# tgialoimtr/cnn_lstm_ctc_ocr

Hardware: AMD Instinct MI355X
Metric: line-crops/sec (train step) at 32x256 bs=256; CER vs ref (higher is better)
Workload: dtype bf16

## Files before the change

cnn_lstm_ctc_ocr_amd/_lib.py:

```python
import ctypes
import os

import torch

_HERE = os.path.dirname(os.path.abspath(__file__))
LIB_PATH = os.environ.get("OCRK_LIB") or os.path.join(_HERE, "libocrk.so")

OCRK_OK = 0
OCRK_ERR_INVALID_ARG = 1
OCRK_ERR_HIP = 2
OCRK_ERR_INFEASIBLE = 3

F32 = 0
BF16 = 1

_p = ctypes.c_void_p
_i32 = ctypes.c_int
_u32 = ctypes.c_uint
_i64 = ctypes.c_int64
_f32 = ctypes.c_float
_sz = ctypes.c_size_t

SIGNATURES = {
    "ocrk_version": [],
# ... 90 lines not shown
    "ocrk_lstm_fwd_persistent_f32": [_p, _p, _p, _i32, _i32, _i32, _p, _p, _p, _p, _p, _p, _p, _sz, _p],
    "ocrk_lstm_bwd_persistent_f32_supported": [_i32, _i32],
    "ocrk_lstm_bwd_persistent_f32_workspace_size": [_i32, _i32],
    "ocrk_lstm_bwd_persistent_f32": [_p, _p, _i32, _i32, _i32, _p, _p, _p, _p, _p, _p, _p, _p, _sz, _p],
    "ocrk_lstm_bwd_persistent_supported": [_i32, _i32],
    "ocrk_lstm_bwd_persistent_workspace_size": [_i32, _i32],
    "ocrk_lstm_bwd_persistent_slices": [_i32, _i32],
    "ocrk_lstm_bwd_persistent": [_p, _p, _i32, _i32, _i32, _p, _p, _p, _p, _p, _p, _p, _p, _sz, _p],
    "ocrk_lstm_fwd": [_p, _p, _p, _p, _p, _i32, _i32, _i32, _p, _p, _p, _p, _i32, _p],
    "ocrk_lstm_bwd": [_p, _p, _p, _p, _i32, _i32, _i32, _p, _p, _p, _p, _i32, _p],
    "ocrk_gemm_workspace_size": [_i32, _i32, _i32, _i32],
    "ocrk_gemm": [_i32, _i32, _i32, _i32, _i32, _f32, _p, _i64, _i64, _p, _i64, _i64, _p, _i64, _i64,
                  _i32, _p, _i32, _i32, _i32, _i32, _i32, _p, _sz, _p],
    "ocrk_adam": [_p, _p, _p, _p, _i64, _f32, _f32, _f32, _f32, _f32, _p],
    "ocrk_adam_ex": [_p, _p, _p, _p, _i64, _f32, _f32, _f32, _f32, _f32, _u32, _p],
    "ocrk_cast": [_p, _i32, _p, _i32, _i64, _p],
    "ocrk_split_bf16": [_p, _i64, _p, _p, _p],
    "ocrk_permute3": [_p, _i32, _i32, _i32, _i32, _p, _i32, _p],
    "ocrk_strided_copy": [_p, _i64, _i64, _i64, _i64, _p, _i32, _i64, _i64, _p],
    "ocrk_colsum_workspace_size": [_i64, _i32],
    "ocrk_colsum": [_p, _i64, _i32, _i32, _p, _i32, _p, _sz, _p],
    "ocrk_slab_sum_workspace_size": [_i32],
    "ocrk_slab_sum": [_p, _i32, _i32, _i32, _p, _i32, _p, _sz, _p],
    "ocrk_relu_mask": [_p, _p, _i64, _f32, _p, _i32, _p],
    "ocrk_mul_scalar": [_p, _i64, _p, _p],
    "ocrk_mean": [_p, _i32, _p, _p],
    "ocrk_seq_len": [_p, _i32, _p, _p],
    "ocrk_timer_create": [_p],
    "ocrk_timer_record": [_p, _p],
    "ocrk_timer_elapsed": [_p, _p, _p],
    "ocrk_timer_destroy": [_p],
}
_RESTYPE = {"ocrk_last_error": ctypes.c_char_p}
_RESTYPE.update({n: ctypes.c_size_t for n in SIGNATURES if n.endswith("_workspace_size")})
_RESTYPE["ocrk_conv_stats_tiles"] = ctypes.c_size_t
_RESTYPE["ocrk_persistent_flags_size"] = ctypes.c_size_t
_RESTYPE["ocrk_bn_bwd_bias_slab_rows"] = ctypes.c_size_t
_RESTYPE["ocrk_bn_bwd_pooled_bias_slab_rows"] = ctypes.c_size_t
_RESTYPE["ocrk_crc32c"] = ctypes.c_uint32


class OcrkError(RuntimeError):

    def __init__(self, status, message):
        super().__init__(message)
        self.status = status
# ... 122 lines not shown
```

cnn_lstm_ctc_ocr_amd/csrc/tensor_ops.hip:

```cpp
#include "common.h"
#include "reduce.h"
#include "mfma_util.h"

template <typename TI, typename TO>
__global__ void __launch_bounds__(256) cast_kernel(const TI* __restrict__ in, TO* __restrict__ out, int64_t n) {
    for (int64_t i = (int64_t)blockIdx.x * 256 + threadIdx.x; i < n; i += (int64_t)gridDim.x * 256)
        out[i] = from_f32<TO>(to_f32(in[i]));
}

template <typename TI, typename TO>
__global__ void __launch_bounds__(256) permute3_kernel(const TI* __restrict__ in, int d0, int d1, int d2,
                                                       TO* __restrict__ out) {
    const int64_t n = (int64_t)d0 * d1 * d2;
    for (int64_t o = (int64_t)blockIdx.x * 256 + threadIdx.x; o < n; o += (int64_t)gridDim.x * 256) {
        int i2 = (int)(o % d2);
        int64_t t = o / d2;
        int i0 = (int)(t % d0);
        int i1 = (int)(t / d0);
        out[o] = from_f32<TO>(to_f32(in[((int64_t)i0 * d1 + i1) * d2 + i2]));
    }
}

namespace ocrk {
namespace {

__global__ void __launch_bounds__(256)
slab_sum_fused(const float* __restrict__ slab, int nslab, int NC, int ld, float* __restrict__ res,
               float* __restrict__ dst_lo, float* __restrict__ dst_hi, int split, int accumulate) {
    constexpr int RG = 64, CQ = 4, U = 16;
    __shared__ double red[RG][4 * CQ + 1];
    const int cq = threadIdx.x % CQ, rg = threadIdx.x / CQ;
    const int c0 = blockIdx.x * 4 * CQ + 4 * cq;
    double s[4] = {0.0, 0.0, 0.0, 0.0};
    if (c0 < NC) {
        const float* col = slab + c0;
        int i = rg;
        for (; i + (U - 1) * RG < nslab; i += U * RG) {
            f32x4 v[U];
#pragma unroll
            for (int u = 0; u < U; ++u) v[u] = *reinterpret_cast<const f32x4*>(col + (int64_t)(i + u * RG) * ld);
#pragma unroll
            for (int u = 0; u < U; ++u)
#pragma unroll
                for (int e = 0; e < 4; ++e) s[e] += v[u][e];
        }
        for (; i < nslab; i += RG) {
            const f32x4 v = *reinterpret_cast<const f32x4*>(col + (int64_t)i * ld);
#pragma unroll
            for (int e = 0; e < 4; ++e) s[e] += v[e];
        }
    }
#pragma unroll
    for (int e = 0; e < 4; ++e) red[rg][4 * cq + e] = s[e];
    __syncthreads();
    if (threadIdx.x < 4 * CQ) {
        const int c = blockIdx.x * 4 * CQ + threadIdx.x;
        if (c >= NC) return;
        double t = 0.0;
        for (int y = 0; y < RG; ++y) t += red[y][threadIdx.x];
        const float v = (float)t;
        if (res) res[c] = v;
        float* d = c < split ? (dst_lo ? dst_lo + c : nullptr) : (dst_hi ? dst_hi + (c - split) : nullptr);
        if (d) *d = accumulate ? *d + v : v;
    }
}

__global__ void __launch_bounds__(256)
slab_sum_stage1(const float* __restrict__ slab, int nslab, int NC, int ld, double* __restrict__ part) {
    __shared__ double red[4][64];
    const int cl = threadIdx.x & 63, q = threadIdx.x >> 6;
    const int c = blockIdx.x * 64 + cl;
    const int rows = (nslab + SLAB_P - 1) / SLAB_P;
    const int r0 = blockIdx.y * rows, r1 = min(nslab, r0 + rows);
    double s = 0.0;
    if (c < NC)
        for (int i = r0 + q; i < r1; i += 4) s += slab[(int64_t)i * ld + c];
    red[q][cl] = s;
    __syncthreads();
    if (q == 0 && c < NC) part[(int64_t)blockIdx.y * NC + c] = red[0][cl] + red[1][cl] + red[2][cl] + red[3][cl];
}

__global__ void __launch_bounds__(64)
slab_sum_stage2(const double* __restrict__ part, int NC, float* __restrict__ res, float* __restrict__ dst_lo,
                float* __restrict__ dst_hi, int split, int accumulate) {
    const int c = blockIdx.x * 64 + threadIdx.x;
    if (c >= NC) return;
    double t = 0.0;
// ... 124 lines not shown
    int64_t rpb = ocrk::cdiv(M, nb);
    nb = std::max<int64_t>(1, ocrk::cdiv(M, rpb));
    hipStream_t s = ocrk::as_stream(stream);
    dim3 grid(colsum_col_blocks(N), (unsigned)nb);
    if (dtype == OCRK_BF16) colsum_partial_kernel<bf16><<<grid, 256, 0, s>>>((const bf16*)in, M, N, rpb, (float*)ws);
    else colsum_partial_kernel<float><<<grid, 256, 0, s>>>((const float*)in, M, N, rpb, (float*)ws);
    int st = ocrk::launch_status("ocrk_colsum");
    if (st) return st;
    double* part = (double*)((char*)ws + ((size_t)nb * N * sizeof(float) + 7) / 8 * 8);
    return ocrk::slab_sum((const float*)ws, (int)nb, N, part, nullptr, out, nullptr, N, accumulate, s);
}

extern "C" size_t ocrk_slab_sum_workspace_size(int nc) { return (size_t)ocrk::SLAB_P * std::max(nc, 1) * sizeof(double); }

extern "C" int ocrk_slab_sum(const float* slab, int nslab, int nc, int ld, float* out, int accumulate, void* ws,
                             size_t ws_bytes, void* stream) {
    OCRK_REQUIRE(nslab >= 0 && nc >= 0 && ld >= nc, "ocrk_slab_sum: bad sizes");
    OCRK_REQUIRE(ws_bytes >= ocrk_slab_sum_workspace_size(nc), "ocrk_slab_sum: workspace too small");
    if (nc == 0) return OCRK_OK;
    return ocrk::slab_sum(slab, nslab, nc, (double*)ws, nullptr, out, nullptr, nc, accumulate, ocrk::as_stream(stream),
                          ld);
}

extern "C" int ocrk_relu_mask(const float* dy, const float* y, int64_t n, float scale, void* out, int out_dtype,
                              void* stream) {
    if (n == 0) return OCRK_OK;
    hipStream_t s = ocrk::as_stream(stream);
    if (out_dtype == OCRK_BF16) relu_mask_kernel<bf16><<<grid1d(n), 256, 0, s>>>(dy, y, n, scale, (bf16*)out);
    else relu_mask_kernel<float><<<grid1d(n), 256, 0, s>>>(dy, y, n, scale, (float*)out);
    return ocrk::launch_status("ocrk_relu_mask");
}

template <typename TO>
__global__ void __launch_bounds__(256) strided_copy_kernel(const float* __restrict__ in, int64_t rows, int64_t cols,
                                                           int64_t in_rs, int64_t in_cs, TO* __restrict__ out,
                                                           int64_t out_rs, int64_t out_cs) {
    const int64_t n = rows * cols;
    for (int64_t i = (int64_t)blockIdx.x * 256 + threadIdx.x; i < n; i += (int64_t)gridDim.x * 256) {
        int64_t r = i / cols, c = i - r * cols;
        out[r * out_rs + c * out_cs] = from_f32<TO>(in[r * in_rs + c * in_cs]);
    }
}

extern "C" int ocrk_strided_copy(const float* in, int64_t rows, int64_t cols, int64_t in_rs, int64_t in_cs,
                                 void* out, int out_dtype, int64_t out_rs, int64_t out_cs, void* stream) {
    int64_t n = rows * cols;
// ... 164 lines not shown
```

cnn_lstm_ctc_ocr_amd/kernels.py:

```python
import ctypes

import torch

from . import _lib, options
from ._lib import ptr, call

F32, BF16 = _lib.F32, _lib.BF16
_DT = {torch.float32: F32, torch.bfloat16: BF16}


def dtype_code(dt):
    try:
        return _DT[dt]
    except KeyError:
        raise TypeError(f"unsupported dtype {dt}; libocrk computes in float32 or bfloat16")


def _stream(t):
    return _lib.stream_ptr(t.device)


def _chk(*ts):
    for t in ts:
        if t is None:
# ... 139 lines not shown
    _chk(x, w_nk, bias, stats)
    B, H, W, Cin = x.shape
    Cout = w_nk.shape[0]
    y_dtype = y_dtype or x.dtype
    y = torch.empty(B, H, W, Cout, dtype=y_dtype, device=x.device)
    call("ocrk_conv3x3_fwd", ptr(x), B, H, W, Cin, ptr(w_nk), ptr(bias), Cout, ptr(y), dtype_code(y_dtype),
         int(relu), ptr(stats), dtype_code(x.dtype), _stream(x))
    return y


def conv3x3_bwd_data(dy, w_bwd, relu_mask=None, dbias=None, accumulate=True, defer=None, relu_bits=None):
    _chk(dy, w_bwd, relu_mask, dbias, relu_bits)
    B, H, W, Cout = dy.shape
    Cin = w_bwd.shape[0]
    dx = torch.empty(B, H, W, Cin, dtype=dy.dtype, device=dy.device)
    if relu_bits is not None:
        if relu_mask is not None:
            raise ValueError("relu_bits replaces relu_mask")
        if dbias is not None and defer is not None:
            tiles = conv_stats_tiles(B * H * W)
            slab = torch.empty(tiles, 2 * Cin, dtype=torch.float32, device=dy.device)
            call("ocrk_conv3x3_bwd_data_bits_slab", ptr(dy), B, H, W, Cout, ptr(w_bwd), Cin, ptr(dx), ptr(relu_bits),
                 ptr(slab), dtype_code(dy.dtype), _stream(dy))
            defer.append((lambda: slab_sum(slab, tiles, Cin, 2 * Cin, dbias, accumulate), (slab,)))
            return dx
        nb, ws = 0, None
        if dbias is not None:
            nb = _lib.lib().ocrk_conv3x3_bwd_data_workspace_size(B, H, W, Cin)
            ws = _ws(nb, dy.device)
        call("ocrk_conv3x3_bwd_data_bits", ptr(dy), B, H, W, Cout, ptr(w_bwd), Cin, ptr(dx), ptr(relu_bits),
             ptr(dbias), int(accumulate), ptr(ws), nb, dtype_code(dy.dtype), _stream(dy))
        return dx
    if dbias is not None and defer is not None:
        tiles = conv_stats_tiles(B * H * W)
        slab = torch.empty(tiles, 2 * Cin, dtype=torch.float32, device=dy.device)
        call("ocrk_conv3x3_bwd_data_slab", ptr(dy), B, H, W, Cout, ptr(w_bwd), Cin, ptr(dx), ptr(relu_mask),
             ptr(slab), dtype_code(dy.dtype), _stream(dy))
        defer.append((lambda: slab_sum(slab, tiles, Cin, 2 * Cin, dbias, accumulate), (slab,)))
        return dx
    nb, ws = 0, None
    if dbias is not None:
        nb = _lib.lib().ocrk_conv3x3_bwd_data_workspace_size(B, H, W, Cin)
        ws = _ws(nb, dy.device)
    call("ocrk_conv3x3_bwd_data", ptr(dy), B, H, W, Cout, ptr(w_bwd), Cin, ptr(dx), ptr(relu_mask), ptr(dbias),
         int(accumulate), ptr(ws), nb, dtype_code(dy.dtype), _stream(dy))
    return dx


def conv3x3_bwd_weight(x, dy, dw, accumulate=True):
    _chk(x, dy, dw)
    B, H, W, Cin = x.shape
    Cout = dy.shape[-1]
    nb = _lib.lib().ocrk_conv3x3_wgrad_workspace_size(B, H, W, Cin, Cout)
    ws = _ws(nb, x.device)
    call("ocrk_conv3x3_bwd_weight", ptr(x), ptr(dy), B, H, W, Cin, Cout, ptr(dw), int(accumulate), ptr(ws), nb,
         dtype_code(x.dtype), _stream(x))


def bn_finalize(stats, M, C, eps, momentum, moving_mean=None, moving_var=None, tile_rows=128):
    _chk(stats, moving_mean, moving_var)
    tiles = stats.shape[0]
# ... 66 lines not shown
                     dbias=None, defer=None, sync=None, pooled=None):
    _chk(z, dp, mean, invstd, gamma, beta, dgamma, dbeta, dbias, pooled)
    B, H, W, C = z.shape
    kh, kw, sh, sw = pool
    nb = _lib.lib().ocrk_bn_bwd_workspace_size(B, H, W, C)
    ws = _ws(nb, z.device)
    dz = torch.empty_like(z)
    if sync is not None:
        return _bn_bwd_sync(z, dp, mean, invstd, gamma, beta, pool, dp_time_major, dgamma, dbeta, accumulate, dbias,
                            defer, sync, dz, ws, nb)
    if pooled is not None:
        if pooled.shape != dp.shape or pooled.dtype != dp.dtype:
            raise ValueError("pooled must have dp's shape and dtype")
        rows = _lib.lib().ocrk_bn_bwd_pooled_bias_slab_rows(B, H, W, C, kh, kw, sh, sw)
        if rows == 0:
            pooled = None
    if pooled is not None:
        slab = None
        if dbias is not None and defer is not None:
            slab = torch.empty(rows, 2 * C, dtype=torch.float32, device=z.device)
        call("ocrk_bn_relu_pool_bwd_pooled", ptr(z), ptr(pooled), ptr(dp), B, H, W, C, ptr(mean), ptr(invstd),
             ptr(gamma), ptr(beta), kh, kw, sh, sw, int(dp_time_major), ptr(dz), ptr(dgamma), ptr(dbeta),
             ptr(dbias), int(accumulate), ptr(slab), ptr(ws), nb, dtype_code(z.dtype), _stream(z))
        if slab is not None:
            def _late():
                slab_sum(slab, rows, C, 2 * C, dbias, accumulate)
                slab_sum(slab.view(-1)[C:], rows, C, 2 * C, dgamma, accumulate)
            defer.append((_late, (slab,)))
        return dz
    if dbias is not None and defer is not None:
        rows = _lib.lib().ocrk_bn_bwd_bias_slab_rows(B, H, W, C, kh, kw, sh, sw)
        slab = torch.empty(rows, C, dtype=torch.float32, device=z.device)
        call("ocrk_bn_relu_pool_bwd_slab", ptr(z), ptr(dp), B, H, W, C, ptr(mean), ptr(invstd), ptr(gamma),
             ptr(beta), kh, kw, sh, sw, int(dp_time_major), ptr(dz), ptr(dgamma), ptr(dbeta), int(accumulate),
             ptr(slab), ptr(ws), nb, dtype_code(z.dtype), _stream(z))
        defer.append((lambda: slab_sum(slab, rows, C, C, dbias, accumulate), (slab,)))
        return dz
    call("ocrk_bn_relu_pool_bwd", ptr(z), ptr(dp), B, H, W, C, ptr(mean), ptr(invstd), ptr(gamma), ptr(beta),
         kh, kw, sh, sw, int(dp_time_major), ptr(dz), ptr(dgamma), ptr(dbeta), ptr(dbias), int(accumulate),
         ptr(ws), nb,
         dtype_code(z.dtype), _stream(z))
    return dz


def _bn_bwd_sync(z, dp, mean, invstd, gamma, beta, pool, dp_time_major, dgamma, dbeta, accumulate, dbias, defer,
                 sync, dz, ws, nb):
    import torch.distributed as dist
    group, count = sync
    B, H, W, C = z.shape
    kh, kw, sh, sw = pool
    dsum = torch.empty(2 * C, dtype=torch.float32, device=z.device)
    args = (ptr(z), ptr(dp), B, H, W, C, ptr(mean), ptr(invstd), ptr(gamma), ptr(beta), kh, kw, sh, sw,
            int(dp_time_major))
    call("ocrk_bn_relu_pool_bwd_reduce", *args, ptr(dgamma), ptr(dbeta), int(accumulate), ptr(dsum), ptr(ws), nb,
         dtype_code(z.dtype), _stream(z))
    dist.all_reduce(dsum, op=dist.ReduceOp.SUM, group=group)
    slab = None
    if dbias is not None and defer is not None:
        rows = _lib.lib().ocrk_bn_bwd_bias_slab_rows(B, H, W, C, kh, kw, sh, sw)
        slab = torch.empty(rows, C, dtype=torch.float32, device=z.device)
    call("ocrk_bn_relu_pool_bwd_apply", *args, ptr(dsum), ptr(count), ptr(dz),
         ptr(dbias if slab is None else None), int(accumulate), ptr(slab), ptr(ws), nb, dtype_code(z.dtype), _stream(z))
    if slab is not None:
        defer.append((lambda: slab_sum(slab, rows, C, C, dbias, accumulate), (slab,)))
    return dz


def gemm(a, b, trans_a=False, trans_b=False, bias=None, relu=False, out=None, out_dtype=torch.float32,
         accumulate=False, alpha=1.0, M=None, N=None, K=None, lda=None, ldb=None, ldc=None,
         batch=1, stride_a=0, stride_b=0, stride_c=0, splits=1):
    for t in (a, b, bias, out):
        if t is not None and not t.is_cuda:
            raise ValueError("libocrk ops take device tensors (got a CPU tensor)")
    if M is None:
        _chk(a, b)
        M, K = (a.shape[1], a.shape[0]) if trans_a else (a.shape[0], a.shape[1])
        N = b.shape[0] if trans_b else b.shape[1]
        lda, ldb = a.shape[1], b.shape[1]
    if out is None:
        out = torch.empty(M, N, dtype=out_dtype, device=a.device)
        ldc = N
    ldc = ldc if ldc is not None else N
    if a.dtype != b.dtype:
        raise TypeError("gemm operands must share a dtype")
    kc = -(-(-(-K // splits)) // 32) * 32 if splits > 1 else K
    splits = -(-K // kc) if splits > 1 else 1
    nb = _lib.lib().ocrk_gemm_workspace_size(M, N, batch, splits) if splits > 1 else 0
# ... 292 lines not shown
    _chk(table, stream_of)
    call("ocrk_copy_batch", ptr(table), int(njobs), int(total_tiles), _stream(stream_of))


def strided_copy(src, rows, cols, in_rs, in_cs, out, out_rs, out_cs, out_offset=0, in_offset=0):
    _chk(src, out)
    sp = ctypes_offset(src, in_offset)
    op = ctypes_offset(out, out_offset)
    call("ocrk_strided_copy", sp, rows, cols, in_rs, in_cs, op, dtype_code(out.dtype), out_rs, out_cs, _stream(src))


def ctypes_offset(t, elems):
    return ctypes.c_void_p(t.data_ptr() + elems * t.element_size())


def slab_sum(slab, nslab, nc, ld, out, accumulate=True):
    _chk(slab, out)
    nb = _lib.lib().ocrk_slab_sum_workspace_size(nc)
    ws = _ws(nb, slab.device)
    call("ocrk_slab_sum", ptr(slab), int(nslab), int(nc), int(ld), ptr(out), int(accumulate), ptr(ws), nb,
         _stream(slab))


def _bias_parts(part, rows, nc, dbias, defer):
    if defer is None:
        slab_sum(part, rows, nc, nc, dbias)
    else:
        defer.append((lambda: slab_sum(part, rows, nc, nc, dbias), (part,)))


def colsum(x, M, N, out, accumulate=True):
    _chk(x, out)
    nb = _lib.lib().ocrk_colsum_workspace_size(M, N)
    ws = _ws(nb, x.device)
    call("ocrk_colsum", ptr(x), M, N, dtype_code(x.dtype), ptr(out), int(accumulate), ptr(ws), nb, _stream(x))


def relu_mask(dy, y, out_dtype, scale=1.0):
    _chk(dy, y)
    out = torch.empty(dy.shape, dtype=out_dtype, device=dy.device)
    call("ocrk_relu_mask", ptr(dy), ptr(y), dy.numel(), float(scale), ptr(out), dtype_code(out_dtype), _stream(dy))
    return out


def mul_scalar_(x, s):
    _chk(x, s)
    call("ocrk_mul_scalar", ptr(x), x.numel(), ptr(s), _stream(x))
    return x


def mean(x):
# ... 174 lines not shown
```

cnn_lstm_ctc_ocr_amd/model.py:

```python
import contextlib

import numpy as np
import torch
import torch.distributed as dist

from . import kernels as K
from . import options
from .config import BN_EPS, BN_MOMENTUM, INFER, LAYER_PARAMS, POOLS, TRAIN, ModelConfig, rnn_size
from .params import ParamStore

layer_params = LAYER_PARAMS

_DEFAULT = []


@contextlib.contextmanager
def use_store(store):
    _DEFAULT.append(store)
    try:
        yield store
    finally:
        _DEFAULT.pop()


# ... 92 lines not shown
                                             store.stats[pe + "/batch_norm/moving_variance"], BN_EPS)
        p = K.bn_relu_pool_fwd(z, mean, invstd, P[pe + "/batch_norm/gamma"], P[pe + "/batch_norm/beta"],
                               POOLS[even], time_major=(k == 4))
        ctx.store, ctx.k = store, k
        ctx.save_for_backward(x, y_odd, z, mean, invstd, p)
        return p

    @staticmethod
    def backward(ctx, dp):
        with _conv_precision(ctx.exact):
            return _ConvBlock._backward(ctx, dp)

    @staticmethod
    def _backward(ctx, dp):
        store, k = ctx.store, ctx.k
        x, y_odd, z, mean, invstd, pooled = ctx.saved_tensors
        dt = store.cfg.dtype
        P, G = store.params, store.grads
        odd, even = f"conv{2 * k - 1}", f"conv{2 * k}"
        pe, po = f"convnet/{even}", f"convnet/{odd}"
        dp = dp.contiguous()
        if dp.dtype != dt:
            dp = K.cast(dp, dt)
        dz = K.bn_relu_pool_bwd(z, dp, mean, invstd, P[pe + "/batch_norm/gamma"], P[pe + "/batch_norm/beta"],
                                POOLS[even], dp_time_major=(k == 4),
                                dgamma=G[pe + "/batch_norm/gamma"], dbeta=G[pe + "/batch_norm/beta"],
                                dbias=G[pe + "/bias"],
                                sync=ctx.bn_sync,
                                pooled=pooled if ctx.bn_sync is None and ctx.pooled_bn else None)
        B, H, W, C = dz.shape
        if k > 1:
            with _conv_side(store, y_odd, dz, *_conv_late_tensors(store)):
                _conv_late_run(store)
                _conv_wgrad(ctx.exact, y_odd, dz, G[pe + "/kernel"])
        _, w_bwd = store.conv_images(even, dt)
        if ctx.conv12_bwd:
            if store.conv_late:
                with _conv_side(store, *_conv_late_tensors(store)):
                    _conv_late_run(store)
            K.conv12_bwd(dz, w_bwd, x, P["convnet/conv1/kernel"], P["convnet/conv1/bias"], G[pe + "/kernel"],
                         G[po + "/kernel"], G[po + "/bias"], relu_bits=ctx.relu_bits)
            store.join()
            return (None, None, None, None) + (None,) * (len(ctx.needs_input_grad) - 4)
        if ctx.c1_fused and K.conv2_bwd_data_conv1_wgrad_ok(dz, x):
            with _conv_side(store, y_odd, dz, *_conv_late_tensors(store)):
                _conv_late_run(store)
                _conv_wgrad(ctx.exact, y_odd, dz, G[pe + "/kernel"])
            bits = ctx.relu_bits
            K.conv2_bwd_data_conv1_wgrad(dz, w_bwd, None if bits is not None else y_odd, x, G[po + "/kernel"],
                                         G[po + "/bias"], relu_bits=bits)
            store.join()
            return (None, None, None, None) + (None,) * (len(ctx.needs_input_grad) - 4)
        if k > 1 and ctx.relu_bits is not None:
            dy_odd = K.conv3x3_bwd_data(dz, w_bwd, dbias=G[po + "/bias"], relu_bits=ctx.relu_bits)
        else:
            dy_odd = K.conv3x3_bwd_data(dz, w_bwd, relu_mask=y_odd, dbias=G[po + "/bias"] if k > 1 else None)
        dx = None
        if k == 1:
            with _conv_side(store, x, dy_odd, *_conv_late_tensors(store)):
                _conv_late_run(store)
                K.conv1_bwd_weight(x, dy_odd, G[po + "/kernel"], G[po + "/bias"])
            _conv_wgrad(ctx.exact, y_odd, dz, G[pe + "/kernel"])
            store.join()
        else:
            if k > 2 and options.get("CONV_SIDE") and options.get("SIDE_STREAM"):
                store.conv_late.append((lambda x=x, d=dy_odd, dw=G[po + "/kernel"], ex=ctx.exact:
                                        _conv_wgrad(ex, x, d, dw), (x, dy_odd)))
            else:
                with _conv_side(store, x, dy_odd):
                    _conv_wgrad(ctx.exact, x, dy_odd, G[po + "/kernel"])
            if ctx.needs_input_grad[0]:
                _, w_bwd_odd = store.conv_images(odd, dt)
                dx = K.conv3x3_bwd_data(dy_odd, w_bwd_odd)
        return (dx, None, None, None) + (None,) * (len(ctx.needs_input_grad) - 4)


def _bn_group(store):
    g = store.bn_group
    if g is None or not (dist.is_available() and dist.is_initialized()):
# ... 93 lines not shown
    @staticmethod
    def forward(ctx, x, seq_len, store, layer, *variables):
        dt = store.cfg.dtype
        T, B, n_in = x.shape
        H = store.cfg.rnn_sizes[layer - 1]
        wxT, _wx, whT, _wh, bias = store.lstm_images(layer, dt)
        gx = K.gemm(x.view(T * B, n_in), wxT, trans_b=True, bias=bias, out_dtype=dt)
        out, hprev, cprev, acts = K.lstm_fwd(gx, whT, seq_len, T, B, H, dt, save=any(ctx.needs_input_grad))
        ctx.store, ctx.layer, ctx.H = store, layer, H
        ctx.save_for_backward(x, seq_len, hprev, cprev, acts)
        return out

    @staticmethod
    def backward(ctx, dout):
        store, layer, H = ctx.store, ctx.layer, ctx.H
        x, seq_len, hprev, cprev, acts = ctx.saved_tensors
        dt = store.cfg.dtype
        T, B, n_in = x.shape
        G4 = 4 * H
        dout = dout.contiguous()
        if dout.dtype != dt:
            dout = K.cast(dout, dt)
        _wxT, wx, _whT, wh, _bias = store.lstm_images(layer, dt)
        dG = K.lstm_bwd(wh, seq_len, dout, cprev, acts, T, B, H, dbias=store.flat_bias_pair_grad(layer))
        R = T * B
        dx = None
        pre = f"rnn/bdrnn{layer}"
        with side_work(store, x, hprev, dG):
            gf, gb = store.grads[f"{pre}/fw/lstm_cell/kernel"], store.grads[f"{pre}/bw/lstm_cell/kernel"]
            sk = gf.numel()
            if dt == torch.float32 and not K.f32_mode_exact():
                (xh, xl), (hh, hl), (gh, gl) = K.split_bf16(x), K.split_bf16(hprev), K.split_bf16(dG)
                passes = [(xh, hh, gh), (xh, hh, gl), (xl, hl, gh)]
            else:
                passes = [(x, hprev, dG)]
            if gb.data_ptr() == gf.data_ptr() + 4 * sk:
                for _xa, ha, ga in passes:
                    K.gemm(ha.view(R, 2 * H), ga.view(R, 2 * G4), trans_a=True, out=gf[n_in:], accumulate=True,
                           M=H, N=G4, K=R, lda=2 * H, ldb=2 * G4, ldc=G4, batch=2, stride_a=H, stride_b=G4,
                           stride_c=sk, splits=_splits(H, G4, R, batch=2, items=_tn_items(layer)))
                for xa, _ha, ga in passes:
                    K.gemm(xa, ga.view(R, 2 * G4), trans_a=True, out=gf, accumulate=True, M=n_in, N=G4, K=R,
                           lda=n_in, ldb=2 * G4, ldc=G4, batch=2, stride_a=0, stride_b=G4, stride_c=sk,
                           splits=_splits(n_in, G4, R, batch=2, items=_tn_items(layer)))
            else:
                for xa, ha, ga in passes:
                    dg = ga.view(R, 2 * G4)
# ... 14 lines not shown
    @staticmethod
    def forward(ctx, x, seq_len, store, layer, *variables):
        dt = store.cfg.dtype
        T, B, n_in = x.shape
        H = store.cfg.rnn_sizes[layer - 1]
        wxT, _wx, whgT, whcT, _whg, _whc, bias = store.gru_images(layer, dt)
        gx = K.gemm(x.view(T * B, n_in), wxT, trans_b=True, bias=bias, out_dtype=dt)
        out, hprev, rh, acts = K.gru_fwd(gx, whgT, whcT, seq_len, T, B, H, dt)
        ctx.store, ctx.layer, ctx.H = store, layer, H
        ctx.save_for_backward(x, seq_len, hprev, rh, acts)
        return out

    @staticmethod
    def backward(ctx, dout):
        store, layer, H = ctx.store, ctx.layer, ctx.H
        x, seq_len, hprev, rh, acts = ctx.saved_tensors
        dt = store.cfg.dtype
        T, B, n_in = x.shape
        G2, G3 = 2 * H, 3 * H
        dout = dout.contiguous()
        if dout.dtype != dt:
            dout = K.cast(dout, dt)
        _wxT, wx, _whgT, _whcT, whg, whc, _bias = store.gru_images(layer, dt)
        dG = K.gru_bwd(whg, whc, seq_len, dout, hprev, acts, T, B, H, dbias=store.gru_bias_cat_grad(layer))
        pre = f"rnn/bdrnn{layer}"
        R = T * B
        side = side_work(store, x, hprev, rh, dG)
        side.__enter__()
        gf, gb = store.grads[f"{pre}/fw/gru_cell/gates/kernel"], store.grads[f"{pre}/bw/gru_cell/gates/kernel"]
        cf, cb = store.grads[f"{pre}/fw/gru_cell/candidate/kernel"], store.grads[f"{pre}/bw/gru_cell/candidate/kernel"]
        sk = (gb.data_ptr() - gf.data_ptr()) // 4
        batched = sk > 0 and cb.data_ptr() - cf.data_ptr() == 4 * sk
        if batched:
            dg = dG.view(R, 2 * G3)
            hp, rhv = hprev.view(R, 2 * H), rh.view(R, 2 * H)
            K.gemm(x, dg, trans_a=True, out=gf, accumulate=True, M=n_in, N=G2, K=R, lda=n_in, ldb=2 * G3,
                   ldc=G2, batch=2, stride_a=0, stride_b=G3, stride_c=sk, splits=_splits(n_in, G2, R, batch=2, items=_tn_items(layer)))
            K.gemm(hp, dg, trans_a=True, out=gf[n_in:], accumulate=True, M=H, N=G2, K=R, lda=2 * H, ldb=2 * G3,
                   ldc=G2, batch=2, stride_a=H, stride_b=G3, stride_c=sk, splits=_splits(H, G2, R, batch=2, items=_tn_items(layer)))
            K.gemm(x, dg[:, G2:], trans_a=True, out=cf, accumulate=True, M=n_in, N=H, K=R, lda=n_in,
                   ldb=2 * G3, ldc=H, batch=2, stride_a=0, stride_b=G3, stride_c=sk,
                   splits=_splits(n_in, H, R, batch=2, items=_tn_items(layer)))
            K.gemm(rhv, dg[:, G2:], trans_a=True, out=cf[n_in:], accumulate=True, M=H, N=H, K=R, lda=2 * H,
                   ldb=2 * G3, ldc=H, batch=2, stride_a=H, stride_b=G3, stride_c=sk, splits=_splits(H, H, R, batch=2, items=_tn_items(layer)))
        for d, dn in enumerate(() if batched else ("fw", "bw")):
            gk = store.grads[f"{pre}/{dn}/gru_cell/gates/kernel"]
            ck = store.grads[f"{pre}/{dn}/gru_cell/candidate/kernel"]
# ... 217 lines not shown
```

cnn_lstm_ctc_ocr_amd/options.py:

```python
import contextlib
import os

_HOST_DEFAULTS = {
    "LSTM_PERSISTENT": 1,
    "F32_TRAIN_EXACT": 0,
    "SIDE_STREAM": 1,
    "CONV_SIDE": 1,
    "CONV12_FUSED": 1,
    "RELU_BITS": 1,
    "POOLED_BN": 1,
    "CONV1_FUSED": 1,
    "CONV12_BWD": 1,
    "TN_ITEMS": 256,
    "TN_ITEMS_L1": 160,
}
KERNEL_OPTIONS = ("CONV_DIRECT", "CONV_ROWS", "CONV_ROWS_WIDE", "CONV_WGRAD_BLOCKS", "LSTM_SPIN_LIMIT",
                  "PERSIST_LATE", "LSTM_BWD_R16", "CTC_LDS",
                  "PP_PERSIST_NK", "NT_F32_EXACT", "NT_F32_MASK",
                  "NT_F32_X6", "BEAM_WAVE", "BN_BWD_BLOCKS", "BN_ROUTE", "BN_ROUTE_SEG", "BN_ROUTE_NCH", "CONV_TN_ITEMS", "CONV_TN4_ITEMS",
                  "CONV_WGRAD_CUS", "F32_MFMA", "GEMM_NT", "GEMM_NT_STAGED", "GEMM_PP", "GEMM_PPTN", "PP_MIN_N", "GEMM_TN",
                  "LSTM_DMA", "LSTM_BWD_DMA", "LSTM_FWD_R16", "NT_TAP_UNIFORM",
                  "GEMM_W4", "GEMM_W4_LAUNCHES")


def _env_int(name, default):
    v = os.environ.get("OCRK_" + name)
    if v is None or v == "":
        return default
    try:
        return int(v)
    except ValueError:
        raise ValueError(f"OCRK_{name}={v!r}: an integer is expected") from None


_HOST = {k: _env_int(k, d) for k, d in _HOST_DEFAULTS.items()}
# ... 41 lines not shown
```

cnn_lstm_ctc_ocr_amd/params.py:

```python

import numpy as np
import torch

from . import kernels as K
from .config import LAYER_PARAMS, ModelConfig

_ALIGN = 64


def param_shapes(cfg):
    out = []
    cin = 1
    for filters, k, _pad, name, bn in LAYER_PARAMS:
        out.append((f"convnet/{name}/kernel", (k, k, cin, filters), True))
        out.append((f"convnet/{name}/bias", (filters,), True))
        if bn:
            out.append((f"convnet/{name}/batch_norm/gamma", (filters,), True))
            out.append((f"convnet/{name}/batch_norm/beta", (filters,), True))
            out.append((f"convnet/{name}/batch_norm/moving_mean", (filters,), False))
            out.append((f"convnet/{name}/batch_norm/moving_variance", (filters,), False))
        cin = filters
    n_in = cin
    for li, H in enumerate(cfg.rnn_sizes, start=1):
        pre = f"rnn/bdrnn{li}"
        if cfg.cell == "lstm":
            for d in ("fw", "bw"):
                out.append((f"{pre}/{d}/lstm_cell/kernel", (n_in + H, 4 * H), True))
# ... 66 lines not shown
        self.offsets = {}
        sizes = {True: 0, False: 0}
        for name, shape, tr in self.spec:
            n = int(np.prod(shape))
            self.offsets[name] = (tr, sizes[tr], shape)
            sizes[tr] += (n + _ALIGN - 1) // _ALIGN * _ALIGN
        self.n_trainable = sum(int(np.prod(s)) for _, s, tr in self.spec if tr)
        self.flat = torch.zeros(sizes[True], dtype=torch.float32, device=self.device)
        self.flat_grad = torch.zeros_like(self.flat)
        self.flat_stats = torch.zeros(max(sizes[False], _ALIGN), dtype=torch.float32, device=self.device)
        self.params, self.grads, self.stats = {}, {}, {}
        for name, shape, tr in self.spec:
            _, off, _ = self.offsets[name]
            n = int(np.prod(shape))
            if tr:
                self.params[name] = self.flat[off:off + n].view(shape)
                self.grads[name] = self.flat_grad[off:off + n].view(shape)
            else:
                self.stats[name] = self.flat_stats[off:off + n].view(shape)
        self.version = 0
        self._images = {}
        self.pending = []
        self.conv_late = []
        self.bn_group = None
        self.f32_conv_exact = False
        self.load_state_dict(values if values is not None else reference_init(self.cfg, seed))

    def state_dict(self):
        out = {k: v.detach().cpu().numpy().copy() for k, v in self.params.items()}
        out.update({k: v.detach().cpu().numpy().copy() for k, v in self.stats.items()})
        return out

    def load_state_dict(self, values):
        for name, _shape, _tr in self.spec:
            if name not in values:
                raise KeyError(f"missing variable {name}")
            dst = self.params.get(name, self.stats.get(name))
            src = torch.as_tensor(np.asarray(values[name], dtype=np.float32))
            if tuple(src.shape) != tuple(dst.shape):
                raise ValueError(f"{name}: shape {tuple(src.shape)} != {tuple(dst.shape)}")
            dst.copy_(src.to(self.device))
        self.bump()

    def save(self, path):
        np.savez(path, **{k.replace("/", "__"): v for k, v in self.state_dict().items()})

    def load(self, path):
        with np.load(path, allow_pickle=False) as z:
            self.load_state_dict({k.replace("__", "/"): z[k] for k in z.files})

    def zero_grad(self):
        self.join()
        self.flat_grad.zero_()

    def join(self):
        while self.conv_late:
            fn, _tensors = self.conv_late.pop(0)
            fn()
        if self.pending:
            cur = torch.cuda.current_stream(self.device)
            for ev in self.pending:
                K.wait_mark(cur, ev)
            self.pending.clear()

    def bump(self):
        self.version += 1
        self._images.clear()
        self._plan_fresh = False

    def images(self, key, builder):
        plan = self._plan_for(key)
        if plan is not None:
            if not self._plan_fresh:
                K.copy_batch(plan["table"], plan["njobs"], plan["tiles"], self.flat)
                self._plan_fresh = True
            return plan["images"][key]
        img = self._images.get(key)
        if img is None:
            img = builder()
            self._images[key] = img
        return img
# ... 193 lines not shown
```

cnn_lstm_ctc_ocr_amd/train.py:

```python
import collections
import math
import time

import torch
import torch.distributed as dist

from . import _lib
from . import kernels as K
from . import options
from . import model as _model
from .config import TRAIN
from .model import check_feasible_host, convnet_layers, ctc_loss_layer, dense_labels, host_labels, rnn_layers




class GradBuckets:

    def __init__(self, store, group=None, comm=None, force=False):
        self.store, self.group, self.comm, self.force = store, group, comm, bool(force)
        rnn = [off for name, (tr, off, _s) in store.offsets.items() if tr and name.startswith("rnn/")]
        self.split = min(rnn) if rnn else store.flat_grad.numel()
        self.work = None
        self._stream = None
        self._comm_world = comm.info()[0] if comm is not None else None

    def world(self):
        if self.comm is not None:
            return self._comm_world
        if not (dist.is_available() and dist.is_initialized()):
            return 1
        return dist.get_world_size(self.group)

    def active(self):
        return self.world() > 1 or (self.force and (self.comm is not None or
                                                    (dist.is_available() and dist.is_initialized())))

    def _sum_(self, t, async_op=False):
        if self.comm is not None:
            self.comm.allreduce_(t)
            return None
        return dist.all_reduce(t, op=dist.ReduceOp.SUM, group=self.group, async_op=async_op)

    def rnn_ready(self, *_):
        if not self.active() or self.work is not None:
            return
        g = self.store.flat_grad
        if g.is_cuda:
            if self._stream is None:
                self._stream = torch.cuda.Stream(g.device)
            K.fork(self._stream, torch.cuda.current_stream(g.device))
            for ev in self.store.pending:
                K.wait_mark(self._stream, ev)
            with torch.cuda.stream(self._stream):
                self.work = self._sum_(g[self.split:], async_op=True)
                if self.work is None:
                    self.work = "stream"
                g.record_stream(self._stream)
        else:
            self.work = self._sum_(g[self.split:], async_op=True)

    def finish(self):
        if not self.active():
            return 1.0
        world = self.world()
        g = self.store.flat_grad
        if self.work is None:
            self._sum_(g)
        else:
            self._sum_(g[:self.split])
# ... 64 lines not shown
        self.buckets = GradBuckets(store, process_group, comm=comm, force=force_exchange)
        self.overlap_allreduce = True

    def learning_rate(self, step=None):
        step = self.global_step if step is None else step
        e = step / self.decay_steps
        if self.staircase:
            e = math.floor(e)
        return self.base_lr * self.decay_rate ** e

    def _bn_group(self):
        if not self.sync_bn or not (dist.is_available() and dist.is_initialized()):
            return None
        return self.group if self.group is not None else dist.group.WORLD

    def world_size(self):
        if self.buckets.comm is not None:
            return self.buckets.world()
        if dist.is_available() and dist.is_initialized():
            return dist.get_world_size(self.group)
        return 1

    def loss_and_grads(self, image, width, label):
        store = self.store
        if store.cfg.dtype != torch.float32:
            return self._loss_and_grads(image, width, label)
        if options.get("F32_TRAIN_EXACT"):
            with K.f32_exact():
                return self._loss_and_grads(image, width, label)
        prev, store.f32_conv_exact = store.f32_conv_exact, True
        try:
            return self._loss_and_grads(image, width, label)
        finally:
            store.f32_conv_exact = prev

    def _loss_and_grads(self, image, width, label):
        store = self.store
        prev_group, store.bn_group = store.bn_group, self._bn_group()
        try:
            return self._forward_backward(image, width, label)
        finally:
            store.bn_group = prev_group

    def _forward_backward(self, image, width, label):
        store = self.store
        if host_labels(label) and not (isinstance(width, torch.Tensor) and width.is_cuda):
# ... 182 lines not shown
```

include/ocrk.h:

```cpp
#ifndef OCRK_H_
#define OCRK_H_

#include <stddef.h>
#include <stdint.h>

#ifdef __cplusplus
extern "C" {
#endif

#define OCRK_ABI_VERSION 7

enum ocrk_status {
    OCRK_OK = 0,
    OCRK_ERR_INVALID_ARG = 1,
    OCRK_ERR_HIP = 2,
    OCRK_ERR_INFEASIBLE = 3
};

enum ocrk_dtype { OCRK_F32 = 0, OCRK_BF16 = 1 };

int ocrk_set_f32_gemm_mode(int mode);
int ocrk_f32_gemm_exact(void);

enum ocrk_device_status {
// ... 211 lines not shown
int ocrk_gemm(int trans_a, int trans_b, int M, int N, int K, float alpha, const void* A, int64_t lda,
              int64_t stride_a, const void* B, int64_t ldb, int64_t stride_b, void* C, int64_t ldc,
              int64_t stride_c, int c_dtype, const float* bias, int relu, int accumulate, int batch,
              int dtype, int splits, void* ws, size_t ws_bytes, void* stream);

int ocrk_adam(float* p, const float* g, float* m, float* v, int64_t n, float lr_t, float beta1,
              float beta2, float eps, float grad_scale, void* stream);
#define OCRK_ADAM_ZERO_GRAD 1u
int ocrk_adam_ex(float* p, float* g, float* m, float* v, int64_t n, float lr_t, float beta1,
                 float beta2, float eps, float grad_scale, unsigned flags, void* stream);

int ocrk_copy_batch(const void* jobs, int njobs, int64_t total_tiles, void* stream);
int ocrk_cast(const void* in, int in_dtype, void* out, int out_dtype, int64_t n, void* stream);
int ocrk_permute3(const void* in, int in_dtype, int d0, int d1, int d2, void* out, int out_dtype,
                  void* stream);
int ocrk_strided_copy(const float* in, int64_t rows, int64_t cols, int64_t in_rs, int64_t in_cs, void* out,
                      int out_dtype, int64_t out_rs, int64_t out_cs, void* stream);
size_t ocrk_colsum_workspace_size(int64_t M, int N);
int ocrk_colsum(const void* in, int64_t M, int N, int dtype, float* out, int accumulate, void* ws,
                size_t ws_bytes, void* stream);
size_t ocrk_slab_sum_workspace_size(int nc);
int ocrk_slab_sum(const float* slab, int nslab, int nc, int ld, float* out, int accumulate, void* ws,
                  size_t ws_bytes, void* stream);
int ocrk_relu_mask(const float* dy, const float* y, int64_t n, float scale, void* out, int out_dtype,
                   void* stream);
int ocrk_mul_scalar(float* x, int64_t n, const float* s, void* stream);
int ocrk_mean(const float* x, int n, float* out, void* stream);
int ocrk_seq_len(const int* widths, int n, int* out, void* stream);

int ocrk_timer_create(void** ev);
int ocrk_timer_record(void* ev, void* stream);
int ocrk_timer_elapsed(void* ev0, void* ev1, float* ms);
int ocrk_timer_destroy(void* ev);

uint32_t ocrk_crc32c(const void* data, size_t n, uint32_t crc);

#ifdef __cplusplus
}
#endif
#endif
```

Before: 56660.

## Batch deferred bias/BN slab reductions into one grouped kernel launch

Adds a batched slab-sum kernel that takes a table of up to 16 reduction jobs and maps blocks to jobs by prefix offsets. The training step now queues bias and gamma slab reductions from the conv, BN-pool and RNN backward passes instead of launching one kernel each, then flushes them once before the gradient all-reduce or join. The goal is to cut many small kernel launches and Python dispatch overhead in backward. In exchange the reductions finish later, the queue holds slabs alive longer, and unaligned items fall back to per-item launches with async malloc and free.

```diff
diff --git a/cnn_lstm_ctc_ocr_amd/_lib.py b/cnn_lstm_ctc_ocr_amd/_lib.py
--- a/cnn_lstm_ctc_ocr_amd/_lib.py
+++ b/cnn_lstm_ctc_ocr_amd/_lib.py
@@ -136,6 +136,7 @@
     "ocrk_colsum": [_p, _i64, _i32, _i32, _p, _i32, _p, _sz, _p],
     "ocrk_slab_sum_workspace_size": [_i32],
     "ocrk_slab_sum": [_p, _i32, _i32, _i32, _p, _i32, _p, _sz, _p],
+    "ocrk_slab_sum_batch": [_p, _i32, _p],
     "ocrk_relu_mask": [_p, _p, _i64, _f32, _p, _i32, _p],
     "ocrk_mul_scalar": [_p, _i64, _p, _p],
     "ocrk_mean": [_p, _i32, _p, _p],
diff --git a/cnn_lstm_ctc_ocr_amd/csrc/tensor_ops.hip b/cnn_lstm_ctc_ocr_amd/csrc/tensor_ops.hip
--- a/cnn_lstm_ctc_ocr_amd/csrc/tensor_ops.hip
+++ b/cnn_lstm_ctc_ocr_amd/csrc/tensor_ops.hip
@@ -24,13 +24,13 @@
 namespace ocrk {
 namespace {
 
-__global__ void __launch_bounds__(256)
-slab_sum_fused(const float* __restrict__ slab, int nslab, int NC, int ld, float* __restrict__ res,
-               float* __restrict__ dst_lo, float* __restrict__ dst_hi, int split, int accumulate) {
+__device__ __forceinline__ void slab_sum_body(const float* __restrict__ slab, int nslab, int NC, int ld,
+                                              float* __restrict__ res, float* __restrict__ dst_lo,
+                                              float* __restrict__ dst_hi, int split, int accumulate, int bx) {
     constexpr int RG = 64, CQ = 4, U = 16;
     __shared__ double red[RG][4 * CQ + 1];
     const int cq = threadIdx.x % CQ, rg = threadIdx.x / CQ;
-    const int c0 = blockIdx.x * 4 * CQ + 4 * cq;
+    const int c0 = bx * 4 * CQ + 4 * cq;
     double s[4] = {0.0, 0.0, 0.0, 0.0};
     if (c0 < NC) {
         const float* col = slab + c0;
@@ -54,7 +54,7 @@
     for (int e = 0; e < 4; ++e) red[rg][4 * cq + e] = s[e];
     __syncthreads();
     if (threadIdx.x < 4 * CQ) {
-        const int c = blockIdx.x * 4 * CQ + threadIdx.x;
+        const int c = bx * 4 * CQ + threadIdx.x;
         if (c >= NC) return;
         double t = 0.0;
         for (int y = 0; y < RG; ++y) t += red[y][threadIdx.x];
@@ -63,6 +63,27 @@
         float* d = c < split ? (dst_lo ? dst_lo + c : nullptr) : (dst_hi ? dst_hi + (c - split) : nullptr);
         if (d) *d = accumulate ? *d + v : v;
     }
+}
+
+__global__ void __launch_bounds__(256)
+slab_sum_fused(const float* __restrict__ slab, int nslab, int NC, int ld, float* __restrict__ res,
+               float* __restrict__ dst_lo, float* __restrict__ dst_hi, int split, int accumulate) {
+    slab_sum_body(slab, nslab, NC, ld, res, dst_lo, dst_hi, split, accumulate, blockIdx.x);
+}
+
+constexpr int SLAB_BATCH = 16;
+struct SlabBatchArgs {
+    OcrkSlabSumItem item[SLAB_BATCH];
+    int first[SLAB_BATCH + 1];
+    int n;
+};
+
+__global__ void __launch_bounds__(256) slab_sum_batch_kernel(const SlabBatchArgs a) {
+    int k = 0;
+    while (k + 1 < a.n && (int)blockIdx.x >= a.first[k + 1]) ++k;
+    const OcrkSlabSumItem& it = a.item[k];
+    slab_sum_body(it.slab, it.nslab, it.nc, it.ld, nullptr, it.dst_lo, it.dst_hi, it.split, it.accumulate,
+                  (int)blockIdx.x - a.first[k]);
 }
 
 __global__ void __launch_bounds__(256)
@@ -233,6 +254,66 @@
                           ld);
 }
 
+namespace {
+bool slab_dst_overlap(const OcrkSlabSumItem& a, const OcrkSlabSumItem& b) {
+    const float* ra[2][2] = {{a.dst_lo, a.dst_lo ? a.dst_lo + a.split : nullptr},
+                             {a.dst_hi, a.dst_hi ? a.dst_hi + (a.nc - a.split) : nullptr}};
+    const float* rb[2][2] = {{b.dst_lo, b.dst_lo ? b.dst_lo + b.split : nullptr},
+                             {b.dst_hi, b.dst_hi ? b.dst_hi + (b.nc - b.split) : nullptr}};
+    for (auto& x : ra)
+        for (auto& y : rb)
+            if (x[0] && y[0] && x[0] < y[1] && y[0] < x[1]) return true;
+    return false;
+}
+
+int slab_batch_launch(ocrk::SlabBatchArgs& a, hipStream_t s) {
+    if (a.n == 0) return OCRK_OK;
+    ocrk::slab_sum_batch_kernel<<<a.first[a.n], 256, 0, s>>>(a);
+    a.n = 0;
+    return ocrk::launch_status("ocrk_slab_sum_batch");
+}
+}
+
+extern "C" int ocrk_slab_sum_batch(const OcrkSlabSumItem* items, int n, void* stream) {
+    OCRK_REQUIRE(n >= 0 && (items || n == 0), "ocrk_slab_sum_batch: n=%d items without a table", n);
+    for (int i = 0; i < n; ++i) {
+        const OcrkSlabSumItem& it = items[i];
+        OCRK_REQUIRE(it.nslab >= 0 && it.nc >= 0 && it.ld >= it.nc && it.split >= 0 && it.split <= it.nc,
+                     "ocrk_slab_sum_batch: item %d has bad sizes (nslab=%d nc=%d ld=%d split=%d)", i, it.nslab,
+                     it.nc, it.ld, it.split);
+        OCRK_REQUIRE(it.slab || it.nslab == 0 || it.nc == 0, "ocrk_slab_sum_batch: item %d has no slab", i);
+    }
+    hipStream_t s = ocrk::as_stream(stream);
+    ocrk::SlabBatchArgs a;
+    a.n = 0;
+    a.first[0] = 0;
+    for (int i = 0; i < n; ++i) {
+        const OcrkSlabSumItem& it = items[i];
+        if (it.nc == 0) continue;
+        const bool fused = it.nc % 4 == 0 && it.ld % 4 == 0 && ((uintptr_t)it.slab & 15) == 0;
+        bool close = !fused || a.n == ocrk::SLAB_BATCH;
+        for (int k = 0; k < a.n && !close; ++k) close = slab_dst_overlap(a.item[k], it);
+        if (close) {
+            int st = slab_batch_launch(a, s);
+            if (st) return st;
+        }
+        if (!fused) {
+            double* part = nullptr;
+            if (hipMallocAsync((void**)&part, ocrk_slab_sum_workspace_size(it.nc), s) != hipSuccess)
+                return ocrk::launch_status("ocrk_slab_sum_batch scratch");
+            int st = ocrk::slab_sum(it.slab, it.nslab, it.nc, part, nullptr, it.dst_lo, it.dst_hi, it.split,
+                                    it.accumulate, s, it.ld);
+            if (hipFreeAsync(part, s) != hipSuccess && !st) st = ocrk::launch_status("ocrk_slab_sum_batch scratch");
+            if (st) return st;
+            continue;
+        }
+        a.item[a.n] = it;
+        a.first[a.n + 1] = a.first[a.n] + (it.nc + 15) / 16;
+        ++a.n;
+    }
+    return slab_batch_launch(a, s);
+}
+
 extern "C" int ocrk_relu_mask(const float* dy, const float* y, int64_t n, float scale, void* out, int out_dtype,
                               void* stream) {
     if (n == 0) return OCRK_OK;
diff --git a/cnn_lstm_ctc_ocr_amd/kernels.py b/cnn_lstm_ctc_ocr_amd/kernels.py
--- a/cnn_lstm_ctc_ocr_amd/kernels.py
+++ b/cnn_lstm_ctc_ocr_amd/kernels.py
@@ -185,7 +185,7 @@
             slab = torch.empty(tiles, 2 * Cin, dtype=torch.float32, device=dy.device)
             call("ocrk_conv3x3_bwd_data_bits_slab", ptr(dy), B, H, W, Cout, ptr(w_bwd), Cin, ptr(dx), ptr(relu_bits),
                  ptr(slab), dtype_code(dy.dtype), _stream(dy))
-            defer.append((lambda: slab_sum(slab, tiles, Cin, 2 * Cin, dbias, accumulate), (slab,)))
+            _defer_sum(defer, slab, tiles, Cin, 2 * Cin, dbias, accumulate)
             return dx
         nb, ws = 0, None
         if dbias is not None:
@@ -199,7 +199,7 @@
         slab = torch.empty(tiles, 2 * Cin, dtype=torch.float32, device=dy.device)
         call("ocrk_conv3x3_bwd_data_slab", ptr(dy), B, H, W, Cout, ptr(w_bwd), Cin, ptr(dx), ptr(relu_mask),
              ptr(slab), dtype_code(dy.dtype), _stream(dy))
-        defer.append((lambda: slab_sum(slab, tiles, Cin, 2 * Cin, dbias, accumulate), (slab,)))
+        _defer_sum(defer, slab, tiles, Cin, 2 * Cin, dbias, accumulate)
         return dx
     nb, ws = 0, None
     if dbias is not None:
@@ -312,7 +312,9 @@
         call("ocrk_bn_relu_pool_bwd_pooled", ptr(z), ptr(pooled), ptr(dp), B, H, W, C, ptr(mean), ptr(invstd),
              ptr(gamma), ptr(beta), kh, kw, sh, sw, int(dp_time_major), ptr(dz), ptr(dgamma), ptr(dbeta),
              ptr(dbias), int(accumulate), ptr(slab), ptr(ws), nb, dtype_code(z.dtype), _stream(z))
-        if slab is not None:
+        if isinstance(defer, SlabSumQueue) and slab is not None:
+            defer.add(slab, rows, 2 * C, 2 * C, dbias, accumulate, dst_hi=dgamma, split=C)
+        elif slab is not None:
             def _late():
                 slab_sum(slab, rows, C, 2 * C, dbias, accumulate)
                 slab_sum(slab.view(-1)[C:], rows, C, 2 * C, dgamma, accumulate)
@@ -324,7 +326,7 @@
         call("ocrk_bn_relu_pool_bwd_slab", ptr(z), ptr(dp), B, H, W, C, ptr(mean), ptr(invstd), ptr(gamma),
              ptr(beta), kh, kw, sh, sw, int(dp_time_major), ptr(dz), ptr(dgamma), ptr(dbeta), int(accumulate),
              ptr(slab), ptr(ws), nb, dtype_code(z.dtype), _stream(z))
-        defer.append((lambda: slab_sum(slab, rows, C, C, dbias, accumulate), (slab,)))
+        _defer_sum(defer, slab, rows, C, C, dbias, accumulate)
         return dz
     call("ocrk_bn_relu_pool_bwd", ptr(z), ptr(dp), B, H, W, C, ptr(mean), ptr(invstd), ptr(gamma), ptr(beta),
          kh, kw, sh, sw, int(dp_time_major), ptr(dz), ptr(dgamma), ptr(dbeta), ptr(dbias), int(accumulate),
@@ -352,7 +354,7 @@
     call("ocrk_bn_relu_pool_bwd_apply", *args, ptr(dsum), ptr(count), ptr(dz),
          ptr(dbias if slab is None else None), int(accumulate), ptr(slab), ptr(ws), nb, dtype_code(z.dtype), _stream(z))
     if slab is not None:
-        defer.append((lambda: slab_sum(slab, rows, C, C, dbias, accumulate), (slab,)))
+        _defer_sum(defer, slab, rows, C, C, dbias, accumulate)
     return dz
 
 
@@ -691,11 +693,56 @@
          _stream(slab))
 
 
+class SlabSumItem(ctypes.Structure):
+    _fields_ = [("slab", ctypes.c_void_p), ("nslab", ctypes.c_int), ("nc", ctypes.c_int), ("ld", ctypes.c_int),
+                ("dst_lo", ctypes.c_void_p), ("dst_hi", ctypes.c_void_p), ("split", ctypes.c_int),
+                ("accumulate", ctypes.c_int)]
+
+
+def slab_sum_batch(items):
+    if not items:
+        return
+    table = (SlabSumItem * len(items))()
+    for e, (slab, nslab, nc, ld, dst_lo, dst_hi, split, accumulate) in zip(table, items):
+        _chk(slab, dst_lo, dst_hi)
+        e.slab, e.nslab, e.nc, e.ld = slab.data_ptr(), int(nslab), int(nc), int(ld)
+        e.dst_lo = None if dst_lo is None else dst_lo.data_ptr()
+        e.dst_hi = None if dst_hi is None else dst_hi.data_ptr()
+        e.split, e.accumulate = int(split), int(accumulate)
+    call("ocrk_slab_sum_batch", table, len(items), _stream(items[0][0]))
+
+
+class SlabSumQueue:
+
+    def __init__(self):
+        self.items = []
+
+    def __len__(self):
+        return len(self.items)
+
+    def add(self, slab, nslab, nc, ld, dst_lo, accumulate=True, dst_hi=None, split=None):
+        self.items.append((slab, nslab, nc, ld, dst_lo, dst_hi, nc if split is None else split, accumulate))
+
+    def flush(self):
+        items, self.items = self.items, []
+        slab_sum_batch(items)
+
+    def clear(self):
+        self.items = []
+
+
+def _defer_sum(defer, slab, nslab, nc, ld, dst, accumulate=True):
+    if isinstance(defer, SlabSumQueue):
+        defer.add(slab, nslab, nc, ld, dst, accumulate)
+    else:
+        defer.append((lambda: slab_sum(slab, nslab, nc, ld, dst, accumulate), (slab,)))
+
+
 def _bias_parts(part, rows, nc, dbias, defer):
     if defer is None:
         slab_sum(part, rows, nc, nc, dbias)
     else:
-        defer.append((lambda: slab_sum(part, rows, nc, nc, dbias), (part,)))
+        _defer_sum(defer, part, rows, nc, nc, dbias)
 
 
 def colsum(x, M, N, out, accumulate=True):
diff --git a/cnn_lstm_ctc_ocr_amd/model.py b/cnn_lstm_ctc_ocr_amd/model.py
--- a/cnn_lstm_ctc_ocr_amd/model.py
+++ b/cnn_lstm_ctc_ocr_amd/model.py
@@ -138,11 +138,12 @@
         dp = dp.contiguous()
         if dp.dtype != dt:
             dp = K.cast(dp, dt)
+        late = store.late_defer()
         dz = K.bn_relu_pool_bwd(z, dp, mean, invstd, P[pe + "/batch_norm/gamma"], P[pe + "/batch_norm/beta"],
                                 POOLS[even], dp_time_major=(k == 4),
                                 dgamma=G[pe + "/batch_norm/gamma"], dbeta=G[pe + "/batch_norm/beta"],
                                 dbias=G[pe + "/bias"],
-                                sync=ctx.bn_sync,
+                                defer=late, sync=ctx.bn_sync,
                                 pooled=pooled if ctx.bn_sync is None and ctx.pooled_bn else None)
         B, H, W, C = dz.shape
         if k > 1:
@@ -168,9 +169,10 @@
             store.join()
             return (None, None, None, None) + (None,) * (len(ctx.needs_input_grad) - 4)
         if k > 1 and ctx.relu_bits is not None:
-            dy_odd = K.conv3x3_bwd_data(dz, w_bwd, dbias=G[po + "/bias"], relu_bits=ctx.relu_bits)
+            dy_odd = K.conv3x3_bwd_data(dz, w_bwd, dbias=G[po + "/bias"], relu_bits=ctx.relu_bits, defer=late)
         else:
-            dy_odd = K.conv3x3_bwd_data(dz, w_bwd, relu_mask=y_odd, dbias=G[po + "/bias"] if k > 1 else None)
+            dy_odd = K.conv3x3_bwd_data(dz, w_bwd, relu_mask=y_odd, dbias=G[po + "/bias"] if k > 1 else None,
+                                        defer=late)
         dx = None
         if k == 1:
             with _conv_side(store, x, dy_odd, *_conv_late_tensors(store)):
@@ -310,7 +312,8 @@
         if dout.dtype != dt:
             dout = K.cast(dout, dt)
         _wxT, wx, _whT, wh, _bias = store.lstm_images(layer, dt)
-        dG = K.lstm_bwd(wh, seq_len, dout, cprev, acts, T, B, H, dbias=store.flat_bias_pair_grad(layer))
+        dG = K.lstm_bwd(wh, seq_len, dout, cprev, acts, T, B, H, dbias=store.flat_bias_pair_grad(layer),
+                        defer=store.late_defer())
         R = T * B
         dx = None
         pre = f"rnn/bdrnn{layer}"
@@ -371,7 +374,8 @@
         if dout.dtype != dt:
             dout = K.cast(dout, dt)
         _wxT, wx, _whgT, _whcT, whg, whc, _bias = store.gru_images(layer, dt)
-        dG = K.gru_bwd(whg, whc, seq_len, dout, hprev, acts, T, B, H, dbias=store.gru_bias_cat_grad(layer))
+        dG = K.gru_bwd(whg, whc, seq_len, dout, hprev, acts, T, B, H, dbias=store.gru_bias_cat_grad(layer),
+                       defer=store.late_defer())
         pre = f"rnn/bdrnn{layer}"
         R = T * B
         side = side_work(store, x, hprev, rh, dG)
diff --git a/cnn_lstm_ctc_ocr_amd/options.py b/cnn_lstm_ctc_ocr_amd/options.py
--- a/cnn_lstm_ctc_ocr_amd/options.py
+++ b/cnn_lstm_ctc_ocr_amd/options.py
@@ -11,6 +11,7 @@
     "POOLED_BN": 1,
     "CONV1_FUSED": 1,
     "CONV12_BWD": 1,
+    "LATE_SUM": 1,
     "TN_ITEMS": 256,
     "TN_ITEMS_L1": 160,
 }
diff --git a/cnn_lstm_ctc_ocr_amd/params.py b/cnn_lstm_ctc_ocr_amd/params.py
--- a/cnn_lstm_ctc_ocr_amd/params.py
+++ b/cnn_lstm_ctc_ocr_amd/params.py
@@ -1,8 +1,11 @@
+
+import contextlib
 
 import numpy as np
 import torch
 
 from . import kernels as K
+from . import options
 from .config import LAYER_PARAMS, ModelConfig
 
 _ALIGN = 64
@@ -115,6 +118,8 @@
         self._images = {}
         self.pending = []
         self.conv_late = []
+        self.late_sums = K.SlabSumQueue()
+        self.late_armed = False
         self.bn_group = None
         self.f32_conv_exact = False
         self.load_state_dict(values if values is not None else reference_init(self.cfg, seed))
@@ -146,10 +151,31 @@
         self.join()
         self.flat_grad.zero_()
 
+    @contextlib.contextmanager
+    def late_summing(self):
+        prev, self.late_armed = self.late_armed, bool(options.get("LATE_SUM"))
+        try:
+            yield
+        except BaseException:
+            self.late_sums.clear()
+            raise
+        finally:
+            self.late_armed = prev
+        if not prev:
+            self.flush_late_sums()
+
+    def late_defer(self):
+        return self.late_sums if self.late_armed else None
+
+    def flush_late_sums(self):
+        if len(self.late_sums):
+            self.late_sums.flush()
+
     def join(self):
         while self.conv_late:
             fn, _tensors = self.conv_late.pop(0)
             fn()
+        self.flush_late_sums()
         if self.pending:
             cur = torch.cuda.current_stream(self.device)
             for ev in self.pending:
diff --git a/cnn_lstm_ctc_ocr_amd/train.py b/cnn_lstm_ctc_ocr_amd/train.py
--- a/cnn_lstm_ctc_ocr_amd/train.py
+++ b/cnn_lstm_ctc_ocr_amd/train.py
@@ -46,6 +46,7 @@
         if not self.active() or self.work is not None:
             return
         g = self.store.flat_grad
+        self.store.flush_late_sums()
         if g.is_cuda:
             if self._stream is None:
                 self._stream = torch.cuda.Stream(g.device)
@@ -156,6 +157,10 @@
         return 1
 
     def loss_and_grads(self, image, width, label):
+        with self.store.late_summing():
+            return self._loss_and_grads_policy(image, width, label)
+
+    def _loss_and_grads_policy(self, image, width, label):
         store = self.store
         if store.cfg.dtype != torch.float32:
             return self._loss_and_grads(image, width, label)
diff --git a/include/ocrk.h b/include/ocrk.h
--- a/include/ocrk.h
+++ b/include/ocrk.h
@@ -257,6 +257,15 @@
 size_t ocrk_slab_sum_workspace_size(int nc);
 int ocrk_slab_sum(const float* slab, int nslab, int nc, int ld, float* out, int accumulate, void* ws,
                   size_t ws_bytes, void* stream);
+typedef struct OcrkSlabSumItem {
+    const float* slab;
+    int nslab, nc, ld;
+    float* dst_lo;
+    float* dst_hi;
+    int split;
+    int accumulate;
+} OcrkSlabSumItem;
+int ocrk_slab_sum_batch(const OcrkSlabSumItem* items, int n, void* stream);
 int ocrk_relu_mask(const float* dy, const float* y, int64_t n, float scale, void* out, int out_dtype,
                    void* stream);
 int ocrk_mul_scalar(float* x, int64_t n, const float* s, void* stream);
```

After: 56760 (median of 3 runs). About the same (+0.2%).
